# MeteoSwiss/flexpart

Measured on AMD Instinct MI355X. Metric: particle-steps/sec (whole node) + achieved HBM GB/s, 1e8 particles, higher is better.
Workload: dtype f64

## Files before the change

flexpart_amd/csrc/fpx_device.hpp:

```cpp
#pragma once
#include "fpx_tu.hpp"
#include <hip/hip_runtime.h>
#include <stdint.h>

namespace fpx {
FPX_TU_OPEN

#define K(x) ((R)(x))
#define FPX_DEV __device__ __forceinline__
#define FPX_HD __host__ __device__ __forceinline__

constexpr int kMaxSpec = 5;
constexpr int kMaxNests = 4;
constexpr int kDead = -999999999;

FPX_HD float m_exp(float x) { return expf(x); }
FPX_HD double m_exp(double x) { return exp(x); }
FPX_HD float m_log(float x) { return logf(x); }
FPX_HD double m_log(double x) { return log(x); }
FPX_HD float m_sqrt(float x) { return sqrtf(x); }
FPX_HD double m_sqrt(double x) { return sqrt(x); }
FPX_HD float m_fma(float a, float b, float c) { return fmaf(a, b, c); }
FPX_HD double m_fma(double a, double b, double c) { return fma(a, b, c); }
FPX_HD float m_sin(float x) { return sinf(x); }
// ... 599 lines not shown
  R isigw;
};

struct PlainMath {
  FPX_DEV double expt(double x) const { return m_expp(x); }
  FPX_DEV double logabs(double x) const { return m_log_abs(x); }
  FPX_DEV float expt(float x) const { return m_expp(x); }
  FPX_DEV float logabs(float x) const { return m_logp(x); }
};

template <typename R, typename MS>
FPX_DEV void zeta_powers(R zeta, const MS &M, R &z23, R &zm13) {
  if (sizeof(R) == 8) {
    const R zc = m_max(zeta, K(1.e-37));
    const R lz = M.logabs(zc);
    const R r13 = m_rcbrt(zc);
    const R d1 = ((K(1.) / K(3.)) - K(.33333)) * lz;
    const R e13 = r13 * (K(1.) + d1 * (K(1.) + d1 * (K(0.5) + d1 * K(0.16666666666666666))));
    const R d = ((K(1.) - K(.33333)) - K(0.66666)) * lz;
    const R corr = K(1.) - d * (K(1.) - d * (K(0.5) - d * K(0.16666666666666666)));
    z23 = zeta * e13 * corr;
    zm13 = zeta > K(1.e-3) ? e13 : K(9.9997697441416293);
  } else {
    const R lz = m_logp(zeta);
    z23 = zeta > K(0.) ? m_expp(K(0.66666) * lz) : K(0.);
    zm13 = m_expp(K(-.33333) * (zeta > K(1.e-3) ? lz : m_logp(K(1.e-3))));
  }
}
template <typename MS>
FPX_DEV double m_pow13(double x, const MS &M) {
  if (__builtin_expect(!(x < 1.0e37), 0)) return m_powr(x, 0.33333);
  const double r = m_rcbrt(x);
  const double d = ((1.0 / 3.0) - .33333) * M.logabs(x);
  return (x * (r * r)) * (1.0 - d * (1.0 - d * (0.5 - d * 0.16666666666666666)));
}
template <typename MS>
FPX_DEV float m_pow13(float x, const MS &) { return m_powr(x, 0.33333f); }

template <typename R, typename MS>
FPX_DEV R tlw_unstable(const Turb<R> &T, R z, const MS &M) {
  if (z < m_abs(T.ol)) return K(0.1) * z * m_rcp(T.sigw * (K(0.55) - K(0.38) * m_abs(z * m_rcp(T.ol))));
  if (T.zeta < K(0.1)) return K(0.59) * z * m_rcp(T.sigw);
  return K(0.15) * T.h * m_rcp(T.sigw) * (K(1.) - M.expt(K(-5) * T.zeta));
}

template <typename R, typename MS>
FPX_DEV void sigw_unstable(Turb<R> &T, const MS &M) {
  R z23, zm13;
  zeta_powers(T.zeta, M, z23, zm13);
  T.sigw = m_sqrtp(K(1.2) * (T.wst * T.wst) * (K(1.) - K(.9) * T.zeta) * z23 + (K(1.8) - K(1.4) * T.zeta) * (T.ust * T.ust)) + K(1.e-2);
  T.dsigwdz = K(0.5) * m_rcp(T.sigw * T.h) * (K(-1.4) * (T.ust * T.ust) + (T.wst * T.wst) * (K(0.8) * zm13 - K(1.8) * z23));
}

template <typename R, typename MS = PlainMath>
FPX_DEV void hanna(Turb<R> &T, R z, const MS &M = MS()) {
  if (T.h / m_abs(T.ol) < K(1.)) {
    T.ust = m_max(K(1.e-4), T.ust);
    R corr = z * m_rcp(T.ust);
    T.sigu = K(1.e-2) + K(2.0) * T.ust * M.expt(K(-3.e-4) * corr);
    T.sigw = K(1.3) * T.ust * M.expt(K(-2.e-4) * corr);
    T.dsigwdz = K(-2.e-4) * T.sigw;
    T.sigw = T.sigw + K(1.e-2);
    T.sigv = T.sigw;
    T.tlu = K(0.5) * z * m_rcp(T.sigw * (K(1.) + K(1.5e-3) * corr));
    T.tlv = T.tlu;
    T.tlw = T.tlu;
  } else if (T.ol < K(0.)) {
    T.sigu = K(1.e-2) + T.ust * m_pow13(K(12) - K(0.5) * T.h * m_rcp(T.ol), M);
    T.sigv = T.sigu;
    sigw_unstable(T, M);
    T.tlu = K(0.15) * T.h * m_rcp(T.sigu);
    T.tlv = T.tlu;
    T.tlw = tlw_unstable(T, z, M);
  } else {
    T.sigu = K(1.e-2) + K(2.) * T.ust * (K(1.) - T.zeta);
    T.sigv = K(1.e-2) + K(1.3) * T.ust * (K(1.) - T.zeta);
    T.sigw = T.sigv;
    T.dsigwdz = K(-1.3) * T.ust * m_rcp(T.h);
    T.tlu = K(0.15) * T.h * m_rcp(T.sigu) * m_sqrtp(T.zeta);
    T.tlv = K(0.467) * T.tlu;
    T.tlw = K(0.1) * T.h * m_rcp(T.sigw) * m_pow08(T.zeta);
  }
  T.tlu = m_max(K(10.), T.tlu);
  T.tlv = m_max(K(10.), T.tlv);
  T.tlw = m_max(K(30.), T.tlw);
  if (T.dsigwdz == K(0.)) T.dsigwdz = K(1.e-10);
}

template <typename R>
FPX_DEV void hanna1(Turb<R> &T, R z) {
  if (T.h / m_abs(T.ol) < K(1.)) {
    T.ust = m_max(K(1.e-4), T.ust);
    T.sigu = K(2.0) * T.ust * m_exp(K(-3.e-4) * z / T.ust);
    T.sigu = m_max(T.sigu, K(1.e-5));
    T.sigv = K(1.3) * T.ust * m_exp(K(-2.e-4) * z / T.ust);
    T.sigv = m_max(T.sigv, K(1.e-5));
    T.sigw = T.sigv;
    T.dsigw2dz = K(-6.76e-4) * T.ust * m_exp(K(-4.e-4) * z / T.ust);
    T.tlu = K(0.5) * z / T.sigw / (K(1.) + K(1.5e-3) * z / T.ust);
    T.tlv = T.tlu;
    T.tlw = T.tlu;
  } else if (T.ol < K(0.)) {
    T.sigu = T.ust * m_powr(K(12) - K(0.5) * T.h / T.ol, K(0.33333));
    T.sigu = m_max(T.sigu, K(1.e-6));
    T.sigv = T.sigu;
    if (T.zeta < K(0.03)) {
// ... 22 lines not shown
    T.tlw = tlw_unstable(T, z, PlainMath());
  } else {
    T.sigu = K(2.) * T.ust * (K(1.) - T.zeta);
    T.sigv = K(1.3) * T.ust * (K(1.) - T.zeta);
    T.sigu = m_max(T.sigu, K(1.e-6));
    T.sigv = m_max(T.sigv, K(1.e-6));
    T.sigw = T.sigv;
    T.dsigw2dz = K(3.38) * T.ust * T.ust * (T.zeta - K(1.)) / T.h;
    T.tlu = K(0.15) * T.h / T.sigu * m_sqrt(T.zeta);
    T.tlv = K(0.467) * T.tlu;
    T.tlw = K(0.1) * T.h / T.sigw * m_powr(T.zeta, K(0.8));
  }
  T.tlu = m_max(K(10.), T.tlu);
  T.tlv = m_max(K(10.), T.tlv);
  T.tlw = m_max(K(30.), T.tlw);
}

enum StashSlot {
  S_U, S_V, S_W,
  S_DDX, S_DDY,
  S_DX, S_DY, S_DAW, S_DCW,
  S_UP, S_VP,
  S_UST, S_WST, S_OL, S_TRANS,
  S_RHOAUX,
  S_NPASS,
  S_COUNT_LEAN,
  S_TDEP = S_COUNT_LEAN,
  S_SETCELL,
  S_SET_NUM, S_SET_DQ6, S_SET_V0,
  S_COUNT_AERO64,
  S_RT_TAG = S_COUNT_AERO64, S_RT_RHO1, S_RT_TT1, S_RT_RHO2, S_RT_TT2,
  S_COUNT
};
template <typename R> constexpr int stash_slots(bool lean, bool susp = true) { return lean ? (susp ? (int)S_COUNT_LEAN : (int)S_NPASS) : (sizeof(R) == 8 ? (int)S_COUNT_AERO64 : (int)S_COUNT); }
constexpr int kStashStride = 256;
template <typename R>
struct Stash {
  typedef __attribute__((address_space(3))) volatile R *lds_ptr;
  lds_ptr p;
  lds_tab_ptr tab;
  FPX_DEV double logabs(double x) const { return m_log_abs(x, tab); }
  FPX_DEV double expt(double x) const { return m_exp_tab(x, tab + kLdsExpTabAt); }
  FPX_DEV float logabs(float x) const { return m_logp(x); }
  FPX_DEV float expt(float x) const { return m_expp(x); }
  FPX_DEV R get(int k) const { return p[k * kStashStride]; }
  FPX_DEV void put(int k, R v) const { p[k * kStashStride] = v; }
  FPX_DEV void add(int k, R v) const { p[k * kStashStride] = p[k * kStashStride] + v; }
};

template <typename R>
struct HsInv {
  R ih, iaux;
  int regime;
};
template <typename R>
FPX_DEV HsInv<R> hanna_short_prepare(Turb<R> &T) {
  HsInv<R> I;
  I.ih = m_rcp(T.h);
  if (T.h / m_abs(T.ol) < K(1.)) {
    I.regime = 0;
    T.ust = m_max(K(1.e-4), T.ust);
    I.iaux = m_rcp(T.ust);
  } else if (T.ol < K(0.)) {
    I.regime = 1;
    I.iaux = m_rcp(T.ol);
  } else {
    I.regime = 2;
    I.iaux = K(0.);
  }
  return I;
}

template <typename R, typename ST>
FPX_DEV void hanna_short(Turb<R> &T, R z, const HsInv<R> &I, const ST &S) {
  if (I.regime == 0) {
    const R corr = z * I.iaux;
    T.sigw = K(1.3) * S.expt(K(-2.e-4) * corr);
    T.dsigwdz = K(-2.e-4) * T.sigw;
    T.sigw = T.sigw * S.get(S_UST) + K(1.e-2);
    const R qn = K(1.) + K(1.5e-3) * corr;
    const R in2 = m_rcp(T.sigw * qn);
    T.isigw = in2 * qn;
    T.tlw = K(0.5) * z * in2;
  } else if (I.regime == 1) {
    R z23, zm13;
    zeta_powers(T.zeta, S, z23, zm13);
    const R ust = S.get(S_UST), wst = S.get(S_WST);
    const R ust2 = ust * ust, wst2 = wst * wst;
    T.sigw = m_sqrtp(K(1.2) * wst2 * (K(1.) - K(.9) * T.zeta) * z23 + (K(1.8) - K(1.4) * T.zeta) * ust2) + K(1.e-2);
    const bool low = z < m_abs(S.get(S_OL));
    const R q = low ? K(0.55) - K(0.38) * m_abs(z * I.iaux) : K(1.);
    const R i2 = m_rcp(T.sigw * q);
    const R isig = i2 * q;
    T.isigw = isig;
    T.dsigwdz = K(0.5) * isig * I.ih * (K(-1.4) * ust2 + wst2 * (K(0.8) * zm13 - K(1.8) * z23));
    if (low) T.tlw = K(0.1) * z * i2;
    else if (T.zeta < K(0.1)) T.tlw = K(0.59) * z * isig;
    else T.tlw = K(0.15) * T.h * isig * (K(1.) - S.expt(K(-5) * T.zeta));
  } else {
    const R ust = S.get(S_UST);
    T.sigw = K(1.e-2) + K(1.3) * ust * (K(1.) - T.zeta);
    T.dsigwdz = K(-1.3) * ust * I.ih;
    T.isigw = m_rcp(T.sigw);
    T.tlw = K(0.1) * T.h * T.isigw * m_pow08(T.zeta);
  }
  T.tlu = m_max(K(10.), T.tlu);
  T.tlv = m_max(K(10.), T.tlv);
  T.tlw = m_max(K(30.), T.tlw);
  if (sizeof(R) == 8) { if (__builtin_expect(T.dsigwdz == K(0.), 0)) { asm volatile("" ::: "memory"); T.dsigwdz = K(1.e-10); } }
  else if (T.dsigwdz == K(0.)) T.dsigwdz = K(1.e-10);
}

#define FPX_PI_PAR K(3.14159265)

template <typename R>
FPX_DEV R cuberoot(R x) { return m_sign(m_pow(m_abs(x), K(0.333333333)), x); }

template <typename R>
FPX_DEV R cbl_transition(R h, R ol) {
  R transition = K(1.);
  if (-h / ol < K(15)) transition = m_sin(((-h / ol + K(10.)) / K(10.)) * FPX_PI_PAR) / K(2.) + K(0.5);
  return transition;
}

template <typename R, typename ST>
FPX_DEV void cbl(const ST &S, int ldirect, R wp, R zp, R wt , R ih , R rhoaux , R sigmaw, R irw , R dsigmawdz, R tlw,
                 R &ath, R &bth, int &flagrein) {
  const R usurad2 = K(0.7071067812), usurad2p = K(0.3989422804), C0 = K(3), costluar4 = K(0.66667), eps = K(0.000001);
  const R timedir = (R)ldirect;
  const R z = zp * ih;
  const R w2 = sigmaw * sigmaw;
  const R rtl = m_rsqrt(tlw);
  const R alfa = (K(2.) / C0) * w2 * (rtl * rtl);
  const R wold = timedir * wp;
  const R omz = K(1.) - z;
  const R omz05 = m_sqrtp(omz), omz15 = omz * omz05;
  const R w3 = (K(1.2) * z * omz15 + eps) * wt;
  const R dw3 = (K(1.2) * (omz15 - z * K(1.5) * omz05)) * (wt * ih);
  const R irw2 = irw * irw, irw3 = irw2 * irw;
  const R skew = w3 * irw3;
  const R dskew = irw3 * dw3 - K(3.) * skew * dsigmawdz * irw;
  R fluarw = K(0.), dfluarw = K(0.), xluarw = K(0.), dxluarw = K(0.);
  if (skew != K(0)) {
    R croot, icroot2;
    m_cuberoot_parts(m_abs(skew), croot, icroot2);
    fluarw = costluar4 * m_sign(croot, skew);
    dfluarw = costluar4 * (K(1.) / K(3.)) * icroot2 * dskew;
  }
  const R fluarw2 = fluarw * fluarw;
  const R a1 = K(1.) + fluarw2, a3 = K(3.) + fluarw2;
  const R ffd = K(2.) * fluarw * dfluarw;
  R a105, ia105;
  m_sqrt_rsqrt(a1, a105, ia105);
  if (skew != K(0)) {
    const R a115 = a1 * a105;
    const R ix = m_rcp(a3 * fluarw);
    xluarw = a115 * skew * ix;
    dxluarw = ((K(1.5) * a105 * ffd * skew + a115 * dskew) - xluarw * (K(3.) * dfluarw * a1)) * ix;
  }
  const R r4 = m_fma(xluarw, xluarw, K(4.));
// ... 730 lines not shown
  }
  A.ixp = A.ix + 1; A.jyp = A.jy + 1;
  if (A.jyp >= nyrows) A.jyp = A.jyp - 1;
  if (A.ixp >= nxcols) A.ixp = nxcols - 1;
  {
    const Fld<R> F = fld_of(V, A.ngrid);
    A.h = F.hcell[(long long)A.jy * F.nx + A.ix];
    if (__builtin_expect(V.interpolhmix != 0 && A.ngrid <= 0, 0)) {
      const R ddx = (R)(xt - (double)(R)A.ix), ddy = (R)(yt - (double)(R)A.jy);
      const R rddx = K(1.) - ddx, rddy = K(1.) - ddy;
      const R p1 = rddx * rddy, p2 = ddx * rddy, p3 = rddx * ddy, p4 = ddx * ddy;
      const TimeW<R> W = time_weights(V, itime);
      R h1[2];
#pragma unroll
      for (int k = 0; k < 2; k++) {
        const int m = k == 0 ? V.m1 : V.m2;
        const long long c00 = (long long)A.jy * F.nx + A.ix, c10 = (long long)A.jy * F.nx + A.ixp;
        const long long c01 = (long long)A.jyp * F.nx + A.ix, c11 = (long long)A.jyp * F.nx + A.ixp;
        h1[k] = p1 * F.sfc[(c00 * 2 + m) * 4 + 3] + p2 * F.sfc[(c10 * 2 + m) * 4 + 3] + p3 * F.sfc[(c01 * 2 + m) * 4 + 3] + p4 * F.sfc[(c11 * 2 + m) * 4 + 3];
      }
      A.h = (h1[0] * W.dt2 + h1[1] * W.dt1) * W.dtt;
    }
    if (TROPO) {
      const int nix = A.ngrid > 0 ? (int)lround((double)A.xr) : (int)lround(xt);
      const int njy = A.ngrid > 0 ? (int)lround((double)A.yr) : (int)lround(yt);
      A.tropop = F.tropo[(long long)njy * F.nx + nix];
    }
  }
  return zt / A.h <= K(1.);
}

template <typename R>
struct PblCtx {
  Cell<R> C;
  R ust, wst, ol;
  R transition;
};

template <typename R>
FPX_DEV void pbl_begin(const View<R> &V, double xt, double yt, const TimeW<R> &W, const AdvCtx<R> &A, PblCtx<R> &B) {
  cell_setup(B.C, A.ix, A.jy, A.ixp, A.jyp, A.xr, A.yr);
  Turb<R> T;
  interp_surface(V, fld_of(V, A.ngrid), B.C, W, T);
  B.ust = T.ust; B.wst = T.wst; B.ol = T.ol;
  B.transition = V.cblflag == 1 ? cbl_transition(A.h, T.ol) : K(1.);
}

template <typename R>
struct LoopCtx {
  int ngrid, ix, jy, ixp, jyp;
  R h;
  int itimec, nrand;
  int nsp;
};

template <typename R>
FPX_DEV void adv_begin_known(const View<R> &V, double xt, double yt, int ngrid, R h, LoopCtx<R> &L, R &ddx, R &ddy) {
  int nyrows = V.ny, nxcols = V.nx;
  R xr, yr;
  L.ngrid = ngrid;
  if (ngrid > 0) {
    const NestDesc<R> &N = V.nest[ngrid - 1];
    xr = (R)((xt - (double)N.xl) * (double)N.xres);
    yr = (R)((yt - (double)N.yl) * (double)N.yres);
    L.ix = (int)xr; L.jy = (int)yr;
    nyrows = N.ny; nxcols = N.nx;
  } else {
    xr = (R)xt; yr = (R)yt;
    L.ix = (int)xt; L.jy = (int)yt;
  }
  L.ixp = L.ix + 1; L.jyp = L.jy + 1;
  if (L.jyp >= nyrows) L.jyp = L.jyp - 1;
  if (L.ixp >= nxcols) L.ixp = nxcols - 1;
  L.h = h;
  ddx = xr - (R)L.ix; ddy = yr - (R)L.jy;
}

template <typename R>
FPX_DEV Cell<R> stash_cell(const LoopCtx<R> &L, const Stash<R> &S) {
  Cell<R> C;
  const R ddx = S.get(S_DDX), ddy = S.get(S_DDY);
  const R rddx = K(1.) - ddx, rddy = K(1.) - ddy;
  C.p1 = rddx * rddy; C.p2 = ddx * rddy; C.p3 = rddx * ddy; C.p4 = ddx * ddy;
  C.ix = L.ix; C.jy = L.jy; C.ixp = L.ixp; C.jyp = L.jyp;
  return C;
}

template <typename R>
FPX_DEV void fetch_level_pair(const View<R> &V, const Fld<R> &F, const TimeW<R> &W, const LoopCtx<R> &L, const Stash<R> &S, int indz, R (&lv)[2][5] ) {
  const R ddx = S.get(S_DDX), ddy = S.get(S_DDY);
  const R rddx = K(1.) - ddx, rddy = K(1.) - ddy;
  typedef const R __attribute__((address_space(1))) *gptr;
  if (F.w3t0 && F.r2t0) {
#ifndef FPX_BLEND_CORNERS
#define FPX_BLEND_CORNERS 4
#endif
    constexpr int NB = FPX_BLEND_CORNERS;
    R acc[2][5];
#pragma unroll
    for (int cb = 0; cb < 4; cb += NB) {
      R y3[NB][6], y2[NB][4];
#pragma unroll
      for (int j = 0; j < NB; j++) {
        const int c = cb + j;
        const int jyc = (c & 2) ? L.jyp : L.jy, ixc = (c & 1) ? L.ixp : L.ix;
        const unsigned int cell = (unsigned int)(jyc * F.nx + ixc) * (unsigned int)V.nz + (unsigned int)(indz - 1);
// ... 42 lines not shown
      const gptr p = (gptr)(F.w3 + (size_t)cell * 6);
      const gptr q = (gptr)(F.r2 + (size_t)cell * 4);
#pragma unroll
      for (int k = 0; k < 12; k++) x3[j][k] = p[k];
#pragma unroll
      for (int k = 0; k < 8; k++) x2[j][k] = q[k];
    }
    __builtin_amdgcn_sched_barrier(0);
#pragma unroll
    for (int j = 0; j < NC; j++) {
      const int c = cb + j;
      const R pw = c == 0 ? rddx * rddy : c == 1 ? ddx * rddy : c == 2 ? rddx * ddy : ddx * ddy;
#pragma unroll
      for (int lev = 0; lev < 2; lev++) {
#pragma unroll
        for (int sl = 0; sl < 2; sl++) {
#pragma unroll
          for (int k = 0; k < 3; k++) {
            const R x = x3[j][(lev * 2 + sl) * 3 + k];
            a3[lev][sl][k] = c == 0 ? pw * x : m_fma(pw, x, a3[lev][sl][k]);
          }
#pragma unroll
          for (int k = 0; k < 2; k++) {
            const R x = x2[j][(lev * 2 + sl) * 2 + k];
            a2[lev][sl][k] = c == 0 ? pw * x : m_fma(pw, x, a2[lev][sl][k]);
          }
        }
      }
    }
    __builtin_amdgcn_sched_barrier(0);
    asm volatile("" ::: "memory");
  }
  const bool h1 = V.m1 != 0, h2 = V.m2 != 0;
#pragma unroll
  for (int lev = 0; lev < 2; lev++) {
    R y[5];
#pragma unroll
    for (int k = 0; k < 5; k++) {
      const R y1 = k < 3 ? (h1 ? a3[lev][1][k] : a3[lev][0][k]) : (h1 ? a2[lev][1][k - 3] : a2[lev][0][k - 3]);
      const R y2 = k < 3 ? (h2 ? a3[lev][1][k] : a3[lev][0][k]) : (h2 ? a2[lev][1][k - 3] : a2[lev][0][k - 3]);
      y[k] = (y1 * W.dt2 + y2 * W.dt1) * W.dtt;
    }
#pragma unroll
    for (int k = 0; k < 5; k++) lv[lev][k] = y[k];
  }
}

template <int T>
FPX_DEV bool sw(int runtime) { return T < 0 ? runtime != 0 : T != 0; }

template <typename R, bool DRYDEP, bool SETTLE, int TSW, int CBLF, typename RNG>
FPX_DEV int pbl_pass(const View<R> &V, const R *hgt, const RNG &G, const TimeW<R> &W, int itime, double xt, double yt,
                     R &zt, R &wp, int &ldt, short &icbt, LoopCtx<R> &A, const Stash<R> &S,
                     int &indz_last, Stats *st) {
  const R eps = V.eps;
  const R eps2 = K(1.e-9);
  const R href = K(15.);
  const R h = A.h;
  const Fld<R> F = fld_of(V, A.ngrid);
  int nrand = A.nrand;
  const bool turbswitch = sw<TSW>(V.turbswitch);
  const bool cblflag = sw<CBLF>(V.cblflag == 1);
  const bool turboff = TSW < 0 && V.turboff != 0;
  Turb<R> T;
  T.ust = S.get(S_UST); T.wst = S.get(S_WST); T.ol = S.get(S_OL); T.h = h;
  T.sigw = K(0.); T.dsigw2dz = K(0.); T.dsigwdz = K(0.);

  if (V.method == 1) {
    ldt = min(ldt, abs(V.lsynctime - A.itimec + itime));
    A.itimec = A.itimec + ldt * V.ldirect;
  } else {
    ldt = abs(V.lsynctime);
    A.itimec = itime + V.lsynctime;
  }
  const R dt = (R)ldt;
  T.zeta = zt / h;

  const int indz = find_level(hgt, V.nz, zt);
  const int indzp = indz + 1;
  indz_last = indz;
  R lv[2][5];
  fetch_level_pair(V, F, W, A, S, indz, lv);

  const R dz = m_rcp(hgt[indzp - 1] - hgt[indz - 1]);
  const R dz1 = (zt - hgt[indz - 1]) * dz;
  const R dz2 = (hgt[indzp - 1] - zt) * dz;
  {
    const R u = dz1 * lv[1][0] + dz2 * lv[0][0];
    const R v = dz1 * lv[1][1] + dz2 * lv[0][1];
    S.put(S_U, u); S.put(S_V, v);
    S.put(S_W, dz1 * lv[1][2] + dz2 * lv[0][2]);
    S.add(S_DX, u * dt);
    S.add(S_DY, v * dt);
  }
  {
    const R rhoa = dz1 * lv[1][3] + dz2 * lv[0][3];
    const R rhograd = dz1 * lv[1][4] + dz2 * lv[0][4];
    S.put(S_RHOAUX, rhograd * m_rcp(rhoa));
  }

  if (turbswitch) hanna(T, zt, S); else hanna1(T, zt);
  S.put(S_UST, T.ust);
  T.isigw = m_rcp(T.sigw);

  if (RNG::kCounter) nrand = (nrand + 3) & ~3;
  if (nrand + 1 > V.maxrand) nrand = 1;
  {
    const R g1 = G.at(nrand), g2 = G.at(nrand + 1);
    const R dttlu = dt * m_rcp(T.tlu), dttlv = dt * m_rcp(T.tlv);
    R up = S.get(S_UP), vp = S.get(S_VP);
    if (dttlu < K(.5)) {
      up = (K(1.) - dttlu) * up + g1 * T.sigu * m_sqrtp(K(2.) * dttlu);
    } else {
      R ru = S.expt(-dttlu);
      up = ru * up + g1 * T.sigu * m_sqrtp(K(1.) - ru * ru);
    }
    if (dttlv < K(.5)) {
      vp = (K(1.) - dttlv) * vp + g2 * T.sigv * m_sqrtp(K(2.) * dttlv);
    } else {
      R rv = S.expt(-dttlv);
      vp = rv * vp + g2 * T.sigv * m_sqrtp(K(1.) - rv * rv);
    }
    if (turboff) { up = K(0.); vp = K(0.); }
    S.put(S_UP, up); S.put(S_VP, vp);
    S.add(S_DAW, up * dt);
    S.add(S_DCW, vp * dt);
  }
  nrand = nrand + 2;

  if (nrand + V.ifine > V.maxrand) nrand = 1;
  const R dtf = dt * V.fine;
  const R dtftlw = dtf * m_rcp(T.tlw);
  const bool cbl_on = cblflag && (-h / T.ol > K(5));
  const R sqrt_dtf = m_sqrtp(dtf);
  const HsInv<R> HI = hanna_short_prepare(T);

  FPX_LANES(st, 0);
  unsigned int flip = icbt < 0 ? 0x80000000u : 0u;
  for (int i = 1; i <= V.ifine; i++) {
    R delz;
    FPX_LANES(st, 1);
    if (turbswitch) {
      if (dtftlw < K(.5)) {
        if (cblflag) {
          if (cbl_on) {
            FPX_LANES(st, 2);
            int flagrein = 0;
            nrand = nrand + 1;
            R old_wp_buf = wp, ath, bth;
            cbl(S, V.ldirect, wp, zt, S.get(S_TRANS), HI.ih, S.get(S_RHOAUX), T.sigw, T.isigw, T.dsigwdz, T.tlw, ath, bth, flagrein);
            wp = m_flip(wp + ath * dtf + bth * G.at(nrand) * sqrt_dtf, flip);
            delz = wp * dtf;
            if (__builtin_expect(flagrein == 1, 0)) {
              re_initialize_particle(V.ldirect, G, zt, S.get(S_WST), h, T.sigw, old_wp_buf, nrand, S.get(S_OL));
              wp = old_wp_buf;
              delz = wp * dtf;
              atomicAdd(&st->nan_count, 1ull);
            }
          } else {
            FPX_LANES(st, 3);
            nrand = nrand + 1;
            R ath = -wp * m_rcp(T.tlw) + T.sigw * T.dsigwdz + wp * wp * T.isigw * T.dsigwdz + T.sigw * T.sigw * S.get(S_RHOAUX);
            R bth = T.sigw * G.at(nrand) * m_sqrtp(K(2.) * dtftlw);
            wp = m_flip(wp + ath * dtf + bth, flip);
            delz = wp * dtf;
            if (__builtin_expect(!isfinite(wp), 0)) {
              nrand = nrand + 1;
              wp = T.sigw * G.at(nrand);
              delz = wp * dtf;
              atomicAdd(&st->nan_count2, 1ull);
            }
          }
        } else {
          wp = m_flip((K(1.) - dtftlw) * wp + G.at(nrand + i) * m_sqrtp(K(2.) * dtftlw) + dtf * (T.dsigwdz + S.get(S_RHOAUX) * T.sigw), flip);
          delz = wp * T.sigw * dtf;
        }
      } else {
        FPX_LANES(st, 4);
        R rw = S.expt(-dtftlw);
        wp = m_flip(rw * wp + G.at(nrand + i) * m_sqrtp(K(1.) - rw * rw) + T.tlw * (K(1.) - rw) * (T.dsigwdz + S.get(S_RHOAUX) * T.sigw), flip);
        delz = wp * T.sigw * dtf;
      }
    } else {
      R rw = m_expp(-dtftlw);
      wp = m_flip(rw * wp + G.at(nrand + i) * m_sqrtp(K(1.) - rw * rw) * T.sigw + T.tlw * (K(1.) - rw) * (T.dsigw2dz + S.get(S_RHOAUX) * (T.sigw * T.sigw)), flip);
      delz = wp * dtf;
    }

    if (turboff) { wp = K(0.); delz = K(0.); }

    if (__builtin_expect(m_abs(delz) > h, 0)) delz = m_fmod(delz, h);
    {
      const bool below = delz < -zt, above = !below && delz > (h - zt);
      flip = (below || above) ? 0x80000000u : 0u;
      const R base = zt + delz;
      const R lift = above ? K(2.) * h : K(0.);
      zt = m_flip(base, flip) + lift;
    }
    if (i != V.ifine) {
      T.zeta = zt * HI.ih;
#ifdef FPX_LANE_STATS
      if (HI.regime == 0) FPX_LANES(st, 5); else if (HI.regime == 1) FPX_LANES(st, 6); else FPX_LANES(st, 7);
#endif
      hanna_short(T, zt, HI, S);
    }
  }
  icbt = flip ? (short)-1 : (short)1;
  if (!cblflag) nrand = nrand + V.ifine + 1;
  A.nrand = nrand;

  if (turbswitch)
    ldt = (int)(m_min(m_min(T.tlw, h * m_rcp(m_max(K(2.) * m_abs(wp * T.sigw), K(1.e-5)))), K(0.5) * m_rcp(m_abs(T.dsigwdz))) * V.ctl);
  else
    ldt = (int)(m_min(T.tlw, h * m_rcp(m_max(K(2.) * m_abs(wp), K(1.e-5)))) * V.ctl);
  ldt = max(ldt, V.mintime);

  R w = S.get(S_W);
  if (SETTLE && V.lsettling) {
    if (V.mdomainfill == 0 && S.get(S_SET_NUM) > K(0.)) w = w + get_settling<R, true>(V, hgt, (int)S.get(S_SETCELL), zt, 0, indz, &S);
    S.put(S_W, w);
  }

  zt = zt + w * dt * (R)V.ldirect;
  if (zt >= hgt[V.nz - 1]) zt = hgt[V.nz - 1] - K(100.) * eps;

  const bool end_of_interval = A.itimec == itime + V.lsynctime;
  if (zt > h) {
    if (end_of_interval) {
      return PBL_DONE;
    }
    return PBL_ESCAPED;
  }

  if (DRYDEP && zt < K(2.) * href) S.add(S_TDEP, m_abs(dt));

  if (zt < K(0.)) zt = m_min(h - eps2, K(-1.) * zt);

  if (end_of_interval) return PBL_DONE;
  return PBL_CONTINUE;
}

template <typename R, typename RNG, bool HAVE_TROPO = false, typename LATE = NoLate>
FPX_DEV void above_step(const View<R> &V, const R *hgt, const RNG &G, const TimeW<R> &W, int itime, double xt, double yt,
                        R &zt, R &wp, int &ldt, AdvCtx<R> &A, R &usig, R &vsig, R &wsig, const LATE &late = LATE()) {
  const R eps2 = K(1.e-9);
  const Fld<R> F = fld_of(V, A.ngrid);
  R tropop;
  if (HAVE_TROPO) tropop = A.tropop;
  else {
    const int nix = A.ngrid > 0 ? (int)lround((double)A.xr) : (int)lround(xt);
    const int njy = A.ngrid > 0 ? (int)lround((double)A.yr) : (int)lround(yt);
    tropop = F.tropo[(long long)njy * F.nx + nix];
  }
  Cell<R> C;
  cell_setup(C, A.ix, A.jy, A.ixp, A.jyp, A.xr, A.yr);
  if (V.turbmesoscale == K(0.)) {
    usig = K(0.); vsig = K(0.); wsig = K(0.);
// ... 562 lines not shown
```

flexpart_amd/csrc/fpx_engine.hip:

```cpp
#include <hip/hip_runtime.h>
#include <cstddef>
#include <cstring>
#include <rccl/rccl.h>
#include <rocprim/device/device_radix_sort.hpp>
#include <rocprim/device/device_scan.hpp>
#include <rocprim/device/device_select.hpp>
#include <rocprim/iterator/counting_iterator.hpp>
#include <algorithm>
#include <cmath>
#include <cstdio>
#include <cstring>
#include <string>
#include <vector>

#include "../../include/flexpart_amd.h"
#include "fpx_tu.hpp"
#include "fpx_device.hpp"
#include "fpx_verttransform.hpp"
#include "fpx_calcpar.hpp"
#include "fpx_convect.hpp"
#include "fpx_rng_host.hpp"

namespace fpx {

// ... 418 lines not shown
}
__device__ __forceinline__ int pbl_state(int pk) { return pk & 3; }
__device__ __forceinline__ int pbl_icbt(int pk) { return (pk & 4) ? -1 : 1; }
__device__ __forceinline__ int pbl_indz(int pk) { return (pk >> 3) & 511; }
__device__ __forceinline__ int pbl_ngrid(int pk) { return ((pk >> 12) & 7) - 2; }
__device__ __forceinline__ int pbl_elapsed(int pk) { return (pk >> 15) & 65535; }
static_assert(kMaxNz <= 512 && kMaxNests + 2 <= 7, "pbl_pack field widths");
template <typename R>
struct PblRec {
  PblRecord<R> *rec;
  R *tdep;
};

template <typename R, bool DRYDEP, bool INIT, bool POLAR, bool NEST, bool CAPCHECK>
__device__ __forceinline__ void prep_body(const View<R> &V, const GridP<R> &Gp, Parts<R> &P, const SeqRng &S, const PblRec<R> &Q, long long s, int itime,
                                          unsigned int step, Stats *st, unsigned char *__restrict__ pbl_flag, const R *hgt,
                                          PState<R> &ps, int itramem, unsigned int pid) {
  constexpr bool MOTHER = !POLAR && !NEST;
  Rng<R> G;
  make_rng(V, pid, step, G);
  const bool is_new = INIT && ((itramem == itime) || (itime == 0));
  if (is_new) {
    int nrand_i;
    R dcas = (R)0, dcas1 = (R)0;
    Rng<R> Gi = G;
    if (V.rng_mode == 0) {
      nrand_i = S.nrand_init[pid];
      if (sizeof(R) == 4) { dcas = (R)S.cbl_dcas[pid]; dcas1 = (R)S.cbl_dcas1[pid]; }
      else { dcas = (R)S.cbl_dcas_d[pid]; dcas1 = (R)S.cbl_dcas1_d[pid]; }
    } else {
      Gi.step = step | 0x80000000u;
      nrand_i = V.rng_mode == 1 ? Gi.start_index(0) : 1;
      dcas = (R)(((float)(Gi.bits(1) >> 8) + 0.5f) * (1.0f / 16777216.0f));
      Rng<R> Gn = Gi;
      Gn.mode = 2;
      dcas1 = Gn.at(7);
    }
    initialize_particle(V, hgt, Gi, nrand_i, itime, ps, dcas, dcas1);
    atomicAdd(&st->n_init, 1ull);
  }

  AdvCtx<R> A;
  const TimeW<R> W = time_weights(V, itime);
  const bool in_pbl = adv_begin<R, MOTHER, true>(V, ps.xt, ps.yt, ps.zt, itime, advance_start_index(V, S, G, pid), A);
  if (V.lsettling) A.nsp = settling_species(V, P.npoint[s]);
  if (in_pbl) {
    if (is_new) {
      P.up[s] = ps.up; P.vp[s] = ps.vp; P.wp[s] = ps.wp;
      P.us[s] = ps.usigold; P.vs[s] = ps.vsigold; P.ws[s] = ps.wsigold;
      P.idt[s] = ps.ldt; P.cbt[s] = ps.icbt;
    }
    PblCtx<R> B;
    pbl_begin(V, ps.xt, ps.yt, W, A, B);
    {
      PblRecord<R> &r = Q.rec[s];
      r.v[8] = B.ust; r.v[9] = B.wst; r.v[10] = B.ol; r.v[11] = B.transition;
      r.v[12] = A.h;
      r.i[0] = A.nrand; r.i[2] = pbl_pack(PBL_FRESH, 1, 0, A.ngrid, 0);
    }
    unsigned char cls;
    if (V.cblflag == 1 && V.turbswitch && (-A.h / B.ol > (R)5)) cls = 1;
    else if (A.h / m_abs(B.ol) < (R)1) cls = 3;
    else if (B.ol < (R)0) cls = 2;
    else cls = 4;
    unsigned char bucket = 0;
    if (V.pbl_cost_buckets) {
      const int idt = is_new ? ps.ldt : P.idt[s];
      const int est = abs(V.lsynctime) / max(idt, 1);
      if (V.pbl_cost_buckets == 1) bucket = est >= 128 ? 3 : est >= 64 ? 2 : est >= 32 ? 1 : 0;
      else if (V.pbl_cost_buckets == 2) bucket = est >= 64 ? 1 : 0;
      else bucket = est >= 256 ? 7 : est >= 128 ? 6 : est >= 96 ? 5 : est >= 64 ? 4 : est >= 48 ? 3 : est >= 32 ? 2 : est >= 16 ? 1 : 0;
    }
    pbl_flag[s] = (unsigned char)((cls - 1) * 8 + (7 - bucket));
    return;
  }
  R usig, vsig, wsig;
  pbl_flag[s] = kKeyDone;
  auto late = [&]() {
    if (!is_new) {
      asm volatile("" : "+v"(s));
      ps.usigold = P.us[s]; ps.vsigold = P.vs[s]; ps.wsigold = P.ws[s];
    }
  };
  above_step<R, Rng<R>, true>(V, hgt, G, W, itime, ps.xt, ps.yt, ps.zt, ps.wp, ps.ldt, A, usig, vsig, wsig, late);
  const int nstop = adv_finish<R, Rng<R>, POLAR, MOTHER, NoLate, CAPCHECK>(V, hgt, G, itime, ps, A, usig, vsig, wsig);
  R prob[kMaxSpec];
#pragma unroll
  for (int ks = 0; ks < kMaxSpec; ks++) prob[ks] = (R)0;
  if (is_new) epilogue_store<R, DRYDEP, true>(V, Gp, P, s, itime, itramem, nstop, ps, prob, st);
  else epilogue_store<R, DRYDEP, false>(V, Gp, P, s, itime, itramem, nstop, ps, prob, st);
}

template <typename R, bool DRYDEP, bool INIT, bool POLAR, bool NEST>
__global__ void __launch_bounds__(kBlock, FPX_PREP_TWO_WAVES(INIT, POLAR, NEST, DRYDEP) ? 2 : FPX_PREP_WAVES) k_prep(View<R> V_arg, GridP<R> Gp_arg, Parts<R> P_arg, SeqRng S_arg, PblRec<R> Q_arg, long long numpart, int itime,
                                                 unsigned int step, Stats *st, unsigned char *__restrict__ pbl_flag,
                                                 unsigned int *__restrict__ pbl_count) {
#ifndef FPX_VIEW_BY_VALUE
  struct KArgs { View<R> V; GridP<R> Gp; Parts<R> P; SeqRng S; PblRec<R> Q; };
  const KArgs &ka = *(const KArgs *)(const void *)__builtin_amdgcn_kernarg_segment_ptr();
  const View<R> &V = ka.V; const GridP<R> &Gp = ka.Gp; Parts<R> &P = const_cast<Parts<R> &>(ka.P); const SeqRng &S = ka.S; const PblRec<R> &Q = ka.Q;
  (void)V_arg; (void)Gp_arg; (void)P_arg; (void)S_arg; (void)Q_arg;
#else
  const View<R> &V = V_arg; const GridP<R> &Gp = Gp_arg; Parts<R> &P = P_arg; const SeqRng &S = S_arg; const PblRec<R> &Q = Q_arg;
#endif
  __shared__ R hgt[kMaxNz];
  for (int k = threadIdx.x; k < V.nz; k += blockDim.x) hgt[k] = V.height[k];
  __syncthreads();
  long long s = (long long)blockIdx.x * blockDim.x + threadIdx.x;
  if (s >= numpart) return;
  PState<R> ps;
  const int itra1_in = P.itra1[s];
  ps.xt = P.xt[s]; ps.yt = P.yt[s]; ps.zt = P.zt[s];
  int itramem = P.itramem[s];
  unsigned int pid = P.pid[s];
  {
    int due_key = itra1_in;
// ... 630 lines not shown
#ifdef FPX_LANE_STATS
            t_x = wall_clock64();
#endif
          } else {
            cur = (unsigned int)c0;
            cbase = cur;
            end = min(cur + 64u, nlist_all);
            ahead = pbl_list[min(cur + (unsigned int)lane, nlist_all - 1u)];
          }
        }
      } else
      while (cur >= end && !out_of_chunks) {
        if (__builtin_amdgcn_readfirstlane(cls_out) == 0u) {
          const unsigned int nseg = __builtin_amdgcn_readfirstlane(cls_n), seg = __builtin_amdgcn_readfirstlane(cls_seg);
          const unsigned int kk = (nseg + 63u) >> 6;
          unsigned int c = 0;
          if (lane == 0) c = atomicAdd(blk + 4 + wcls, 1u);
          c = __builtin_amdgcn_readfirstlane(c);
          if (c < kk) {
            cur = seg + c * 64u;
            cbase = cur; FPX_IN_VGPR(cbase);
            end = min(cur + 64u, seg + nseg);
            ahead = pbl_list[min(cur + (unsigned int)lane, end - 1u)];
            break;
          }
          cls_out = 1u; FPX_IN_VGPR(cls_out);
        }
        if (can_suspend) {
          const int live = __popcll(__ballot(have));
          if (live > 0 && live >= drain_lanes) break;
          suspend(have);
          need = ~0ull;
        }
        wcls++;
        cls_out = 0u; FPX_IN_VGPR(cls_out);
        if (wcls < 4) { cls_n = mine[wcls]; cls_seg = mine[8 + wcls]; FPX_IN_VGPR(cls_n); FPX_IN_VGPR(cls_seg); }
        if (wcls == 4) {
          out_of_chunks = true;
#ifdef FPX_LANE_STATS
          t_x = wall_clock64();
#endif
        }
      }
      if (cur < end) {
        const unsigned int rank = __popcll(need & ((1ull << lane) - 1ull));
        const unsigned int my = cur + rank;
        const unsigned int s_new = (unsigned int)__builtin_amdgcn_ds_bpermute((int)(min(my - cbase, 63u) << 2), (int)ahead);
        if (!have && my < end) {
          FPX_LANES(st, 8);
          s = s_new;
          const PblRecord<R> *rp = Q.rec + s;
          const double l_xt = P.xt[s], l_yt = P.yt[s];
          const unsigned int l_pid = P.pid[s];
          const int r_nrand = rp->i[0], r_ldt = SUSP ? rp->i[1] : 0, r_pk = rp->i[2];
          const R r_ust = rp->v[8], r_wst = rp->v[9], r_ol = rp->v[10], r_trans = rp->v[11], r_h = rp->v[12];
          R l_zt = P.zt[s], l_wp = P.wp[s], l_up = P.up[s], l_vp = P.vp[s];
          int l_idt = P.idt[s];
          short l_cbt = P.cbt[s];
          const R c_dx = SUSP ? rp->v[0] : (R)0, c_dy = SUSP ? rp->v[1] : (R)0, c_daw = SUSP ? rp->v[2] : (R)0, c_dcw = SUSP ? rp->v[3] : (R)0;
          const R c_zt = SUSP ? rp->v[4] : (R)0, c_up = SUSP ? rp->v[5] : (R)0, c_vp = SUSP ? rp->v[6] : (R)0, c_wp = SUSP ? rp->v[7] : (R)0;
          int l_npoint = 0;
          if (!LEAN && V.lsettling) l_npoint = P.npoint[s];
          R c_tdep = (R)0;
          if (SUSP && !LEAN && V.drydep) c_tdep = Q.tdep[s];
          __builtin_amdgcn_sched_barrier(0);
          const bool resumed = SUSP && pbl_state(r_pk) == PBL_CONTINUE;
          xt = l_xt; yt = l_yt; pid = l_pid;
          zt = resumed ? c_zt : l_zt; wp = resumed ? c_wp : l_wp;
          ldt = resumed ? r_ldt : l_idt;
          icbt = resumed ? (short)pbl_icbt(r_pk) : l_cbt;
          {
            R ddx, ddy;
            adv_begin_known(V, xt, yt, pbl_ngrid(r_pk), r_h, A, ddx, ddy);
            A.itimec = SUSP ? itime + pbl_elapsed(r_pk) * V.ldirect : itime;
            A.nrand = r_nrand;
            A.nsp = 0;
            if (!LEAN && V.lsettling) {
              const int nsp = settling_species(V, l_npoint);
              const SettleSpec<R> sp = settle_spec(V, nsp);
              S.put(S_SET_NUM, spec_row(V, nsp).density > (R)0 ? sp.num : (R)0);
              S.put(S_SET_DQ6, sp.dq6); S.put(S_SET_V0, sp.vset);
              S.put(S_SETCELL, (R)settling_column(V, (R)xt, (R)yt));
              if (sizeof(R) == 4) S.put(S_RT_TAG, (R)0);
            }
            S.put(S_DDX, ddx); S.put(S_DDY, ddy);
          }
          S.put(S_DX, resumed ? c_dx : (R)0); S.put(S_DY, resumed ? c_dy : (R)0);
          S.put(S_DAW, resumed ? c_daw : (R)0); S.put(S_DCW, resumed ? c_dcw : (R)0);
          S.put(S_W, (R)0);
          S.put(S_UP, resumed ? c_up : l_up); S.put(S_VP, resumed ? c_vp : l_vp);
          S.put(S_UST, r_ust); S.put(S_WST, r_wst); S.put(S_OL, r_ol);
          S.put(S_TRANS, (r_wst * r_wst * r_wst) * r_trans);
          if (SUSP) S.put(S_NPASS, (R)0);
          if (!LEAN && V.drydep) S.put(S_TDEP, resumed ? c_tdep : (R)0);
          have = true;
        }
        cur = min(cur + (unsigned int)__popcll(need), end);
      }
    }
    if (!__any(have)) {
      if (out_of_chunks) break;
      continue;
    }
    bool over_budget = false;
    if (have) {
      Rng<R, RNGM> G;
      make_rng(V, pid, step, G);
      int indz = 1;
      const int rc = pbl_pass<R, !LEAN, !LEAN, TSW, CBLF>(V, hgt, G, W, itime, xt, yt, zt, wp, ldt, icbt, A, S, indz, st);
      R npass = (R)0;
      if (SUSP) { npass = S.get(S_NPASS) + (R)1; S.put(S_NPASS, npass); }
      if (rc != PBL_CONTINUE) {
        FPX_LANES(st, 9);
        write_record(rc, indz);
        have = false;
      } else over_budget = SUSP && npass >= cap_r;
    }
    if (SUSP && cap_passes > 0) suspend(over_budget);
  }
#ifdef FPX_LANE_STATS
  if (lane == 0) {
    const unsigned long long t_e = wall_clock64();
    atomicAdd(&st->lanes[11][0], 1ull);
    atomicAdd(&st->lanes[11][1], t_x - t_s);
    atomicAdd(&st->lanes[12][0], t_e - t_s);
    atomicMax(&st->lanes[12][1], t_e - t_s);
    atomicMax(&st->lanes[13][0], ~(t_x - t_s));
    atomicMax(&st->lanes[13][1], t_e - t_x);
  }
#endif
}

__global__ void k_math_probe(int fn, const double *__restrict__ x, double *__restrict__ y, long long n) {
  const long long i = (long long)blockIdx.x * blockDim.x + threadIdx.x;
  if (i >= n) return;
  const double v = x[i];
  double r = 0.0, c, ic2;
  switch (fn) {
    case 0: r = m_expp(v); break;
    case 1: r = m_logp(v); break;
    case 2: r = m_sqrtp(v); break;
    case 3: r = m_rcp(v); break;
    case 4: r = m_rsqrt(v); break;
    case 5: m_cuberoot_parts(v, c, ic2); r = c; break;
    case 7: r = m_erf_e(v, m_expp(-(v * v))); break;
    case 8: r = m_pow08(v); break;
    case 9: r = m_exp_tab(v, &kExpTab[0]); break;
    case 10: r = m_log_abs(v); break;
    case 11: r = m_rcbrt(v); break;
    default: m_cuberoot_parts(v, c, ic2); r = ic2; break;
  }
  y[i] = r;
}

template <typename R, bool DRYDEP, bool POLAR, bool NEST, bool CAPCHECK>
__device__ __forceinline__ void finish_body(const View<R> &V, const GridP<R> &Gp, Parts<R> &P, unsigned int s, const PblRecord<R> &rec, R tdep,
                                            int itime, unsigned int step, Stats *st, const R *hgt, DryDep<R> *dry) {
  constexpr bool MOTHER = !POLAR && !NEST;
  const int pk = rec.i[2];
  PState<R> ps;
  ps.xt = P.xt[s]; ps.yt = P.yt[s]; ps.zt = rec.v[4];
  ps.up = rec.v[5]; ps.vp = rec.v[6]; ps.wp = rec.v[7];
// ... 3909 lines not shown
```

Before: 375.5 million.

## Precompute per-particle turbulence invariants once and reuse them in PBL passes

Computes the stability regime, reciprocals of h, ol and ust, and the unstable-regime sigu and 1/tlu once per particle in the setup stage and stores them in the PBL record. Each pass reloads them instead of redoing divisions and the cube root. A new hanna overload returns inverse Lagrangian timescales, and the Langevin update becomes FMA-based and shares factors when tlu equals tlv. Squared ust and wst are passed into hanna_short in lean variants. In exchange, record slots v[0..3] and i[1] are now shared with the suspend state, which needs a recompute on resume and adds extra global reads and writes.

```diff
diff --git a/flexpart_amd/csrc/fpx_device.hpp b/flexpart_amd/csrc/fpx_device.hpp
--- a/flexpart_amd/csrc/fpx_device.hpp
+++ b/flexpart_amd/csrc/fpx_device.hpp
@@ -675,6 +675,75 @@
   T.dsigwdz = K(0.5) * m_rcp(T.sigw * T.h) * (K(-1.4) * (T.ust * T.ust) + (T.wst * T.wst) * (K(0.8) * zm13 - K(1.8) * z23));
 }
 
+enum { INV_NEUTRAL = 0, INV_UNSTABLE = 1, INV_STABLE = 2, INV_REGIME = 3,
+       INV_CBL = 4 };
+template <typename R>
+struct StepInv {
+  R ih, iaux;
+  R sigu, itlu;
+  int flags;
+};
+template <typename R>
+FPX_DEV int step_regime(R h, R ol) {
+  const R hol = h / ol;
+  const int regime = m_abs(hol) < K(1.) ? INV_NEUTRAL : ol < K(0.) ? INV_UNSTABLE : INV_STABLE;
+  return regime | (-hol > K(5) ? INV_CBL : 0);
+}
+template <typename R, typename MS>
+FPX_DEV StepInv<R> step_invariants(R h, R ol, R ust, const MS &M) {
+  StepInv<R> I;
+  I.flags = step_regime(h, ol);
+  I.ih = m_rcp(h);
+  I.iaux = K(0.); I.sigu = K(0.); I.itlu = K(0.);
+  const int regime = I.flags & INV_REGIME;
+  if (regime == INV_NEUTRAL) {
+    I.iaux = m_rcp(m_max(K(1.e-4), ust));
+  } else if (regime == INV_UNSTABLE) {
+    I.iaux = m_rcp(ol);
+    I.sigu = m_fma(ust, m_pow13(m_fma(-(K(0.5) * h), I.iaux, K(12)), M), K(1.e-2));
+    I.itlu = m_rcp(m_max(K(10.), K(0.15) * h * m_rcp(I.sigu)));
+  }
+  return I;
+}
+
+template <typename R, typename MS>
+FPX_DEV void hanna(Turb<R> &T, R z, const StepInv<R> &I, const MS &M, R &itlu, R &itlv, bool &same_tl) {
+  const int regime = I.flags & INV_REGIME;
+  same_tl = true;
+  if (regime == INV_NEUTRAL) {
+    R corr = z * I.iaux;
+    T.sigu = K(1.e-2) + K(2.0) * T.ust * M.expt(K(-3.e-4) * corr);
+    T.sigw = K(1.3) * T.ust * M.expt(K(-2.e-4) * corr);
+    T.dsigwdz = K(-2.e-4) * T.sigw;
+    T.sigw = T.sigw + K(1.e-2);
+    T.sigv = T.sigw;
+    T.tlu = K(0.5) * z * m_rcp(T.sigw * (K(1.) + K(1.5e-3) * corr));
+    T.tlw = T.tlu;
+    itlu = m_rcp(m_max(K(10.), T.tlu));
+    itlv = itlu;
+  } else if (regime == INV_UNSTABLE) {
+    T.sigu = I.sigu;
+    T.sigv = T.sigu;
+    sigw_unstable(T, M);
+    T.tlw = tlw_unstable(T, z, M);
+    itlu = I.itlu;
+    itlv = itlu;
+  } else {
+    T.sigu = K(1.e-2) + K(2.) * T.ust * (K(1.) - T.zeta);
+    T.sigv = K(1.e-2) + K(1.3) * T.ust * (K(1.) - T.zeta);
+    T.sigw = T.sigv;
+    T.dsigwdz = K(-1.3) * T.ust * I.ih;
+    T.tlu = K(0.15) * T.h * m_rcp(T.sigu) * m_sqrtp(T.zeta);
+    T.tlv = K(0.467) * T.tlu;
+    T.tlw = K(0.1) * T.h * m_rcp(T.sigw) * m_pow08(T.zeta);
+    itlu = m_rcp(m_max(K(10.), T.tlu));
+    itlv = m_rcp(m_max(K(10.), T.tlv));
+    same_tl = false;
+  }
+  T.tlw = m_max(K(30.), T.tlw);
+  if (T.dsigwdz == K(0.)) T.dsigwdz = K(1.e-10);
+}
+
 template <typename R, typename MS = PlainMath>
 FPX_DEV void hanna(Turb<R> &T, R z, const MS &M = MS()) {
   if (T.h / m_abs(T.ol) < K(1.)) {
@@ -803,26 +872,16 @@
 struct HsInv {
   R ih, iaux;
   int regime;
+  R ust2, wst2;
 };
 template <typename R>
-FPX_DEV HsInv<R> hanna_short_prepare(Turb<R> &T) {
+FPX_DEV HsInv<R> hanna_short_prepare(const StepInv<R> &J) {
   HsInv<R> I;
-  I.ih = m_rcp(T.h);
-  if (T.h / m_abs(T.ol) < K(1.)) {
-    I.regime = 0;
-    T.ust = m_max(K(1.e-4), T.ust);
-    I.iaux = m_rcp(T.ust);
-  } else if (T.ol < K(0.)) {
-    I.regime = 1;
-    I.iaux = m_rcp(T.ol);
-  } else {
-    I.regime = 2;
-    I.iaux = K(0.);
-  }
+  I.ih = J.ih; I.iaux = J.iaux; I.regime = J.flags & INV_REGIME;
   return I;
 }
 
-template <typename R, typename ST>
+template <bool SQ, typename R, typename ST>
 FPX_DEV void hanna_short(Turb<R> &T, R z, const HsInv<R> &I, const ST &S) {
   if (I.regime == 0) {
     const R corr = z * I.iaux;
@@ -836,8 +895,11 @@
   } else if (I.regime == 1) {
     R z23, zm13;
     zeta_powers(T.zeta, S, z23, zm13);
-    const R ust = S.get(S_UST), wst = S.get(S_WST);
-    const R ust2 = ust * ust, wst2 = wst * wst;
+    R ust2 = I.ust2, wst2 = I.wst2;
+    if (!SQ) {
+      const R ust = S.get(S_UST), wst = S.get(S_WST);
+      ust2 = ust * ust; wst2 = wst * wst;
+    }
     T.sigw = m_sqrtp(K(1.2) * wst2 * (K(1.) - K(.9) * T.zeta) * z23 + (K(1.8) - K(1.4) * T.zeta) * ust2) + K(1.e-2);
     const bool low = z < m_abs(S.get(S_OL));
     const R q = low ? K(0.55) - K(0.38) * m_abs(z * I.iaux) : K(1.);
@@ -855,8 +917,6 @@
     T.isigw = m_rcp(T.sigw);
     T.tlw = K(0.1) * T.h * T.isigw * m_pow08(T.zeta);
   }
-  T.tlu = m_max(K(10.), T.tlu);
-  T.tlv = m_max(K(10.), T.tlv);
   T.tlw = m_max(K(30.), T.tlw);
   if (sizeof(R) == 8) { if (__builtin_expect(T.dsigwdz == K(0.), 0)) { asm volatile("" ::: "memory"); T.dsigwdz = K(1.e-10); } }
   else if (T.dsigwdz == K(0.)) T.dsigwdz = K(1.e-10);
@@ -1693,6 +1753,7 @@
   R h;
   int itimec, nrand;
   int nsp;
+  int flags;
 };
 
 template <typename R>
@@ -1841,7 +1902,7 @@
 template <typename R, bool DRYDEP, bool SETTLE, int TSW, int CBLF, typename RNG>
 FPX_DEV int pbl_pass(const View<R> &V, const R *hgt, const RNG &G, const TimeW<R> &W, int itime, double xt, double yt,
                      R &zt, R &wp, int &ldt, short &icbt, LoopCtx<R> &A, const Stash<R> &S,
-                     int &indz_last, Stats *st) {
+                     int &indz_last, Stats *st, const R *inv4 ) {
   const R eps = V.eps;
   const R eps2 = K(1.e-9);
   const R href = K(15.);
@@ -1870,6 +1931,13 @@
   indz_last = indz;
   R lv[2][5];
   fetch_level_pair(V, F, W, A, S, indz, lv);
+  StepInv<R> J;
+  J.flags = A.flags;
+  {
+    typedef const R __attribute__((address_space(1))) *gptr;
+    const gptr q = (gptr)inv4;
+    J.ih = q[0]; J.iaux = q[1]; J.sigu = q[2]; J.itlu = q[3];
+  }
 
   const R dz = m_rcp(hgt[indzp - 1] - hgt[indz - 1]);
   const R dz1 = (zt - hgt[indz - 1]) * dz;
@@ -1888,27 +1956,52 @@
     S.put(S_RHOAUX, rhograd * m_rcp(rhoa));
   }
 
-  if (turbswitch) hanna(T, zt, S); else hanna1(T, zt);
-  S.put(S_UST, T.ust);
+  R itlu, itlv;
+  bool same_tl = false;
+  if (turbswitch) hanna(T, zt, J, S, itlu, itlv, same_tl);
+  else {
+    hanna1(T, zt);
+    itlu = m_rcp(T.tlu); itlv = m_rcp(T.tlv);
+  }
   T.isigw = m_rcp(T.sigw);
 
   if (RNG::kCounter) nrand = (nrand + 3) & ~3;
   if (nrand + 1 > V.maxrand) nrand = 1;
   {
     const R g1 = G.at(nrand), g2 = G.at(nrand + 1);
-    const R dttlu = dt * m_rcp(T.tlu), dttlv = dt * m_rcp(T.tlv);
     R up = S.get(S_UP), vp = S.get(S_VP);
-    if (dttlu < K(.5)) {
-      up = (K(1.) - dttlu) * up + g1 * T.sigu * m_sqrtp(K(2.) * dttlu);
+    const R dttlu = dt * itlu;
+    if (sizeof(R) == 8 && TSW >= 0) {
+      auto factors = [&](R dttl, R &mem, R &amp) {
+        if (dttl < K(.5)) {
+          mem = K(1.) - dttl;
+          amp = m_sqrtp(K(2.) * dttl);
+        } else {
+          mem = S.expt(-dttl);
+          amp = m_sqrtp(K(1.) - mem * mem);
+        }
+      };
+      R memu, ampu;
+      factors(dttlu, memu, ampu);
+      R memv = memu, ampv = ampu;
+      if (!same_tl) factors(dt * itlv, memv, ampv);
+      if (dttlu < K(.5)) up = m_fma(g1 * T.sigu, ampu, memu * up);
+      else up = m_fma(memu, up, g1 * T.sigu * ampu);
+      vp = m_fma(memv, vp, g2 * T.sigv * ampv);
     } else {
-      R ru = S.expt(-dttlu);
-      up = ru * up + g1 * T.sigu * m_sqrtp(K(1.) - ru * ru);
-    }
-    if (dttlv < K(.5)) {
-      vp = (K(1.) - dttlv) * vp + g2 * T.sigv * m_sqrtp(K(2.) * dttlv);
-    } else {
-      R rv = S.expt(-dttlv);
-      vp = rv * vp + g2 * T.sigv * m_sqrtp(K(1.) - rv * rv);
+      const R dttlv = dt * itlv;
+      if (dttlu < K(.5)) {
+        up = (K(1.) - dttlu) * up + g1 * T.sigu * m_sqrtp(K(2.) * dttlu);
+      } else {
+        R ru = S.expt(-dttlu);
+        up = ru * up + g1 * T.sigu * m_sqrtp(K(1.) - ru * ru);
+      }
+      if (dttlv < K(.5)) {
+        vp = (K(1.) - dttlv) * vp + g2 * T.sigv * m_sqrtp(K(2.) * dttlv);
+      } else {
+        R rv = S.expt(-dttlv);
+        vp = rv * vp + g2 * T.sigv * m_sqrtp(K(1.) - rv * rv);
+      }
     }
     if (turboff) { up = K(0.); vp = K(0.); }
     S.put(S_UP, up); S.put(S_VP, vp);
@@ -1920,9 +2013,11 @@
   if (nrand + V.ifine > V.maxrand) nrand = 1;
   const R dtf = dt * V.fine;
   const R dtftlw = dtf * m_rcp(T.tlw);
-  const bool cbl_on = cblflag && (-h / T.ol > K(5));
+  const bool cbl_on = cblflag && (J.flags & INV_CBL) != 0;
   const R sqrt_dtf = m_sqrtp(dtf);
-  const HsInv<R> HI = hanna_short_prepare(T);
+  HsInv<R> HI = hanna_short_prepare(J);
+  constexpr bool SQ = !SETTLE && !DRYDEP && TSW >= 0;
+  HI.ust2 = SQ ? T.ust * T.ust : K(0.); HI.wst2 = SQ ? T.wst * T.wst : K(0.);
 
   FPX_LANES(st, 0);
   unsigned int flip = icbt < 0 ? 0x80000000u : 0u;
@@ -1991,7 +2086,7 @@
 #ifdef FPX_LANE_STATS
       if (HI.regime == 0) FPX_LANES(st, 5); else if (HI.regime == 1) FPX_LANES(st, 6); else FPX_LANES(st, 7);
 #endif
-      hanna_short(T, zt, HI, S);
+      hanna_short<SQ>(T, zt, HI, S);
     }
   }
   icbt = flip ? (short)-1 : (short)1;
diff --git a/flexpart_amd/csrc/fpx_engine.hip b/flexpart_amd/csrc/fpx_engine.hip
--- a/flexpart_amd/csrc/fpx_engine.hip
+++ b/flexpart_amd/csrc/fpx_engine.hip
@@ -494,16 +494,19 @@
     }
     PblCtx<R> B;
     pbl_begin(V, ps.xt, ps.yt, W, A, B);
+    const StepInv<R> J = step_invariants(A.h, B.ol, B.ust, PlainMath());
     {
       PblRecord<R> &r = Q.rec[s];
       r.v[8] = B.ust; r.v[9] = B.wst; r.v[10] = B.ol; r.v[11] = B.transition;
       r.v[12] = A.h;
       r.i[0] = A.nrand; r.i[2] = pbl_pack(PBL_FRESH, 1, 0, A.ngrid, 0);
+      r.v[0] = J.ih; r.v[1] = J.iaux; r.v[2] = J.sigu; r.v[3] = J.itlu;
+      r.i[1] = J.flags;
     }
     unsigned char cls;
-    if (V.cblflag == 1 && V.turbswitch && (-A.h / B.ol > (R)5)) cls = 1;
-    else if (A.h / m_abs(B.ol) < (R)1) cls = 3;
-    else if (B.ol < (R)0) cls = 2;
+    if (V.cblflag == 1 && V.turbswitch && (J.flags & INV_CBL)) cls = 1;
+    else if ((J.flags & INV_REGIME) == INV_NEUTRAL) cls = 3;
+    else if ((J.flags & INV_REGIME) == INV_UNSTABLE) cls = 2;
     else cls = 4;
     unsigned char bucket = 0;
     if (V.pbl_cost_buckets) {
@@ -1240,12 +1243,12 @@
           const PblRecord<R> *rp = Q.rec + s;
           const double l_xt = P.xt[s], l_yt = P.yt[s];
           const unsigned int l_pid = P.pid[s];
-          const int r_nrand = rp->i[0], r_ldt = SUSP ? rp->i[1] : 0, r_pk = rp->i[2];
+          const int r_nrand = rp->i[0], r_i1 = rp->i[1], r_pk = rp->i[2];
           const R r_ust = rp->v[8], r_wst = rp->v[9], r_ol = rp->v[10], r_trans = rp->v[11], r_h = rp->v[12];
           R l_zt = P.zt[s], l_wp = P.wp[s], l_up = P.up[s], l_vp = P.vp[s];
           int l_idt = P.idt[s];
           short l_cbt = P.cbt[s];
-          const R c_dx = SUSP ? rp->v[0] : (R)0, c_dy = SUSP ? rp->v[1] : (R)0, c_daw = SUSP ? rp->v[2] : (R)0, c_dcw = SUSP ? rp->v[3] : (R)0;
+          const R r_v0 = rp->v[0], r_v1 = rp->v[1], r_v2 = rp->v[2], r_v3 = rp->v[3];
           const R c_zt = SUSP ? rp->v[4] : (R)0, c_up = SUSP ? rp->v[5] : (R)0, c_vp = SUSP ? rp->v[6] : (R)0, c_wp = SUSP ? rp->v[7] : (R)0;
           int l_npoint = 0;
           if (!LEAN && V.lsettling) l_npoint = P.npoint[s];
@@ -1255,7 +1258,7 @@
           const bool resumed = SUSP && pbl_state(r_pk) == PBL_CONTINUE;
           xt = l_xt; yt = l_yt; pid = l_pid;
           zt = resumed ? c_zt : l_zt; wp = resumed ? c_wp : l_wp;
-          ldt = resumed ? r_ldt : l_idt;
+          ldt = resumed ? r_i1 : l_idt;
           icbt = resumed ? (short)pbl_icbt(r_pk) : l_cbt;
           {
             R ddx, ddy;
@@ -1263,6 +1266,7 @@
             A.itimec = SUSP ? itime + pbl_elapsed(r_pk) * V.ldirect : itime;
             A.nrand = r_nrand;
             A.nsp = 0;
+            A.flags = resumed ? -1 : r_i1;
             if (!LEAN && V.lsettling) {
               const int nsp = settling_species(V, l_npoint);
               const SettleSpec<R> sp = settle_spec(V, nsp);
@@ -1273,11 +1277,12 @@
             }
             S.put(S_DDX, ddx); S.put(S_DDY, ddy);
           }
-          S.put(S_DX, resumed ? c_dx : (R)0); S.put(S_DY, resumed ? c_dy : (R)0);
-          S.put(S_DAW, resumed ? c_daw : (R)0); S.put(S_DCW, resumed ? c_dcw : (R)0);
+          S.put(S_DX, resumed ? r_v0 : (R)0); S.put(S_DY, resumed ? r_v1 : (R)0);
+          S.put(S_DAW, resumed ? r_v2 : (R)0); S.put(S_DCW, resumed ? r_v3 : (R)0);
           S.put(S_W, (R)0);
           S.put(S_UP, resumed ? c_up : l_up); S.put(S_VP, resumed ? c_vp : l_vp);
-          S.put(S_UST, r_ust); S.put(S_WST, r_wst); S.put(S_OL, r_ol);
+          S.put(S_UST, (A.flags & INV_REGIME) == INV_NEUTRAL ? m_max((R)1.e-4, r_ust) : r_ust);
+          S.put(S_WST, r_wst); S.put(S_OL, r_ol);
           S.put(S_TRANS, (r_wst * r_wst * r_wst) * r_trans);
           if (SUSP) S.put(S_NPASS, (R)0);
           if (!LEAN && V.drydep) S.put(S_TDEP, resumed ? c_tdep : (R)0);
@@ -1286,6 +1291,12 @@
         cur = min(cur + (unsigned int)__popcll(need), end);
       }
     }
+    if (SUSP && have && A.flags < 0) {
+      const StepInv<R> J = step_invariants(A.h, S.get(S_OL), S.get(S_UST), PlainMath());
+      A.flags = J.flags;
+      PblRecord<R> *rp = Q.rec + s;
+      rp->v[0] = J.ih; rp->v[1] = J.iaux; rp->v[2] = J.sigu; rp->v[3] = J.itlu;
+    }
     if (!__any(have)) {
       if (out_of_chunks) break;
       continue;
@@ -1295,7 +1306,7 @@
       Rng<R, RNGM> G;
       make_rng(V, pid, step, G);
       int indz = 1;
-      const int rc = pbl_pass<R, !LEAN, !LEAN, TSW, CBLF>(V, hgt, G, W, itime, xt, yt, zt, wp, ldt, icbt, A, S, indz, st);
+      const int rc = pbl_pass<R, !LEAN, !LEAN, TSW, CBLF>(V, hgt, G, W, itime, xt, yt, zt, wp, ldt, icbt, A, S, indz, st, &Q.rec[s].v[0]);
       R npass = (R)0;
       if (SUSP) { npass = S.get(S_NPASS) + (R)1; S.put(S_NPASS, npass); }
       if (rc != PBL_CONTINUE) {
```

New measurement: 380.9 million (median of 6 runs). 1.01x the previous value.
